# kshedden/muscato

Hardware: AMD Instinct MI355X
Metric: reads/sec (100 bp, multi-map) at 1/2/4/8 MI355X; confirm-kernel HBM GB/s vs peak (higher is better)
Workload: dtype u32

## Files before the change

include/muscato_hip.h:

```cpp
#ifndef MUSCATO_HIP_H
#define MUSCATO_HIP_H

#include <stdint.h>

#ifdef __cplusplus
extern "C" {
#endif

#define MUSC_ABI_VERSION 3
#define MUSC_MAX_WINDOWS 16

typedef struct musc_ctx musc_ctx;

typedef struct {
  uint32_t read_idx;
  uint32_t gene_idx;
  uint32_t pos;
  uint32_t nmiss;
} musc_hit;

typedef struct {
  int32_t n_windows;
  int32_t windows[MUSC_MAX_WINDOWS];
  int32_t window_width;
// ... 96 lines not shown
int musc_results_text(musc_ctx* ctx, uint64_t line0, uint64_t nlines, char* dst, uint64_t capacity, int dst_on_device,
                      uint64_t* nbytes);
int musc_results_last_ms(musc_ctx* ctx, float* ms_order, float* ms_text);
int musc_results_number_key(uint32_t pos, uint32_t nmiss, uint64_t* key);

enum { MUSC_SIDE_NONMATCH = 0, MUSC_SIDE_GENESTATS = 1, MUSC_SIDE_READSTATS = 2 };
int musc_side_prepare(musc_ctx* ctx, uint64_t* nrecords, uint64_t* nbytes);
int musc_side_text(musc_ctx* ctx, int which, uint64_t rec0, uint64_t nrec, char* dst, uint64_t capacity, int dst_on_device,
                   uint64_t* nbytes);
int musc_side_last_ms(musc_ctx* ctx, float* ms_prepare, float* ms_text);

#define MUSC_INSTANCE_WORDS 4
#define MUSC_INST_MATCH_T 1u
#define MUSC_INST_MATCH_G 2u
#define MUSC_INST_SCREEN 3u
#define MUSC_INST_SCREEN_T 4u
#define MUSC_INST_CONFIRM 5u
int musc_last_instance(const musc_ctx* ctx, uint32_t* out);
int musc_instances(uint32_t* out, uint32_t capacity, uint32_t* n);

int musc_stream_plan(uint64_t nreads, uint32_t fixed_len, uint32_t batch_reads, uint64_t* ends, uint8_t* is_batch_end,
                     uint64_t capacity, uint64_t* n, uint64_t* planned_batches);

int musc_overflow_probes(musc_ctx* ctx, uint32_t** read_idx, uint32_t** window, uint64_t* n);
void musc_free_u32(uint32_t* p);

#define MUSC_MM_MAX_READ_LEN 1024
int musc_maxmatches_apply(musc_ctx* ctx, int apply_mmtol, uint64_t* nhits, uint64_t* n_suspect_probes,
                          uint64_t* n_truncated_blocks);
int musc_maxmatches_last_ms(musc_ctx* ctx, float* ms);
int musc_maxmatches_last_detail(musc_ctx* ctx, uint64_t* n_pairs, float* ms_replay);

int musc_gather(musc_ctx* const* ctxs, int n, const uint64_t* read_base, musc_hit** hits,
                uint64_t* nhits);
int musc_gather_rccl(musc_ctx* const* ctxs, int n, const uint64_t* read_base, musc_hit** hits,
                     uint64_t* nhits);
int musc_rccl_probe(char* msg, uint64_t cap);

typedef struct musc_db_text_info {
  uint64_t n_targets, n_bases;
  uint64_t n_odd;
  uint32_t first_odd_target, reserved;
  uint64_t n_text_bytes, n_chunks;
  float ms_decode, ms_parse;
} musc_db_text_info;
int musc_sz_decode(musc_ctx* ctx, const uint8_t* bytes, uint64_t nbytes, uint8_t* dst, uint64_t capacity,
// ... 28 lines not shown
```

muscato_amd/_lib.py:

```python
from __future__ import annotations

import ctypes
import os

HERE = os.path.dirname(os.path.abspath(__file__))
LIB_PATH = os.environ.get("MUSC_LIB_PATH") or os.path.join(HERE, "libmuscato_hip.so")

MUSC_MAX_WINDOWS = 16


class MuscHit(ctypes.Structure):
    _fields_ = [("read_idx", ctypes.c_uint32), ("gene_idx", ctypes.c_uint32),
                ("pos", ctypes.c_uint32), ("nmiss", ctypes.c_uint32)]


class MuscParams(ctypes.Structure):
    _fields_ = [
        ("n_windows", ctypes.c_int32),
        ("windows", ctypes.c_int32 * MUSC_MAX_WINDOWS),
        ("window_width", ctypes.c_int32),
        ("pmatch", ctypes.c_double),
        ("min_dinuc", ctypes.c_int32),
        ("max_read_length", ctypes.c_int32),
        ("max_matches", ctypes.c_int32),
# ... 39 lines not shown
        ("n_targets", ctypes.c_uint64), ("n_bases", ctypes.c_uint64), ("n_odd", ctypes.c_uint64),
        ("first_odd_target", ctypes.c_uint32), ("reserved", ctypes.c_uint32),
        ("n_text_bytes", ctypes.c_uint64), ("n_chunks", ctypes.c_uint64),
        ("ms_decode", ctypes.c_float), ("ms_parse", ctypes.c_float),
    ]


class MuscTargetsPrepInfo(ctypes.Structure):
    _fields_ = [
        ("n_lines", ctypes.c_uint64), ("n_records", ctypes.c_uint64), ("n_targets", ctypes.c_uint64),
        ("n_dropped", ctypes.c_uint64), ("stop_line", ctypes.c_uint64), ("n_subx", ctypes.c_uint64),
        ("n_seq_bytes", ctypes.c_uint64), ("n_id_bytes", ctypes.c_uint64),
        ("ms", ctypes.c_float), ("reserved", ctypes.c_uint32),
    ]


SYMBOLS = [
    "musc_abi_version", "musc_init", "musc_destroy", "musc_last_error", "musc_reload_env",
    "musc_db_load_ascii", "musc_db_load_packed", "musc_db_build_index", "musc_db_build_index_for",
    "musc_db_set_partition_bases", "musc_db_partitions",
    "musc_reads_load_ascii", "musc_reads_load_packed", "musc_reads_load_packed32", "musc_reads_sort_unique",
    "musc_reads_prep_fastq", "musc_fastq_prep_free",
    "musc_match_device", "musc_hits_copy", "musc_hits_copy_packed", "musc_hits_copy_compact", "musc_hits_unpack", "musc_match", "musc_free_hits",
    "musc_get_stats", "musc_last_instance", "musc_instances", "musc_stream_plan", "musc_gather", "musc_gather_rccl", "musc_rccl_probe", "musc_overflow_probes", "musc_free_u32",
    "musc_results_set_gene_text", "musc_results_set_read_text", "musc_results_order", "musc_results_hits", "musc_results_text",
    "musc_results_last_ms", "musc_results_number_key",
    "musc_side_prepare", "musc_side_text", "musc_side_last_ms",
    "musc_maxmatches_apply", "musc_maxmatches_last_ms", "musc_maxmatches_last_detail",
    "musc_sz_decode", "musc_db_load_text",
    "musc_targets_prep", "musc_targets_prep_text", "musc_targets_prep_load", "musc_targets_prep_free", "musc_sz_frame",
]

SIDE_NONMATCH, SIDE_GENESTATS, SIDE_READSTATS = 0, 1, 2

_lib = None


def load() -> ctypes.CDLL:
    global _lib
    if _lib is not None:
        return _lib
    if not os.path.exists(LIB_PATH):
        raise ImportError(
            "muscato_amd: %s is missing -- build it with `python -m muscato_amd.build` "
            "(hipcc, gfx950).  There is no CPU fallback." % LIB_PATH)
    import sys
    torch = sys.modules.get("torch")
# ... 22 lines not shown
    lib.musc_db_set_partition_bases.argtypes = [vp, u64]
    lib.musc_db_partitions.argtypes = [vp, vp, ctypes.c_uint32, ctypes.POINTER(ctypes.c_uint32)]
    lib.musc_reads_load_ascii.argtypes = [vp, vp, vp, u64, ctypes.c_int]
    lib.musc_reads_load_packed.argtypes = [vp, vp, vp, vp, u64]
    lib.musc_reads_load_packed32.argtypes = [vp, vp, vp, vp, ctypes.c_uint32, u64, ctypes.c_int]
    lib.musc_reads_sort_unique.argtypes = [vp, vp, vp, u64, ctypes.c_int, ctypes.POINTER(vp), ctypes.POINTER(vp),
                                           ctypes.POINTER(u64)]
    lib.musc_reads_prep_fastq.argtypes = [vp, vp, u64, ctypes.c_int, i32, i32, ctypes.POINTER(MuscFastqPrep)]
    lib.musc_reads_prep_fastq.restype = ctypes.c_int
    lib.musc_fastq_prep_free.argtypes = [ctypes.POINTER(MuscFastqPrep)]
    lib.musc_fastq_prep_free.restype = None
    lib.musc_match_device.argtypes = [vp, ctypes.POINTER(MuscParams), ctypes.POINTER(u64)]
    lib.musc_hits_copy.argtypes = [vp, vp, u64, ctypes.c_int]
    lib.musc_hits_copy_packed.argtypes = [vp, vp, u64, ctypes.c_int, u64, ctypes.POINTER(i32)]
    lib.musc_hits_copy_compact.argtypes = [vp, vp, u64, vp, u64, ctypes.c_int, ctypes.POINTER(i32)]
    lib.musc_hits_unpack.argtypes = [vp, vp, u64, ctypes.c_int, ctypes.POINTER(i32), vp]
    lib.musc_match.argtypes = [vp, ctypes.POINTER(MuscParams), ctypes.POINTER(vp), ctypes.POINTER(u64)]
    lib.musc_free_hits.argtypes = [vp]
    lib.musc_free_hits.restype = None
    lib.musc_get_stats.argtypes = [vp, ctypes.POINTER(MuscStats)]
    lib.musc_last_instance.argtypes = [vp, ctypes.POINTER(ctypes.c_uint32)]
    lib.musc_instances.argtypes = [ctypes.POINTER(ctypes.c_uint32), ctypes.c_uint32, ctypes.POINTER(ctypes.c_uint32)]
    lib.musc_stream_plan.argtypes = [u64, ctypes.c_uint32, ctypes.c_uint32, vp, vp, u64, ctypes.POINTER(u64), ctypes.POINTER(u64)]
    lib.musc_overflow_probes.argtypes = [vp, ctypes.POINTER(vp), ctypes.POINTER(vp), ctypes.POINTER(u64)]
    lib.musc_overflow_probes.restype = ctypes.c_int
    lib.musc_free_u32.argtypes = [vp]
    lib.musc_free_u32.restype = None
    lib.musc_gather.argtypes = [ctypes.POINTER(vp), ctypes.c_int, ctypes.POINTER(u64),
                                ctypes.POINTER(vp), ctypes.POINTER(u64)]
    lib.musc_gather_rccl.argtypes = lib.musc_gather.argtypes
    lib.musc_rccl_probe.argtypes = [ctypes.c_char_p, ctypes.c_uint64]
    lib.musc_results_set_gene_text.argtypes = [vp, vp, vp, vp, ctypes.c_uint32]
    lib.musc_results_set_read_text.argtypes = [vp, vp, vp, u64]
    lib.musc_results_order.argtypes = [vp, vp, u64, ctypes.c_int, ctypes.POINTER(u64), ctypes.POINTER(u64)]
    lib.musc_results_hits.argtypes = [vp, vp, u64, ctypes.c_int]
    lib.musc_results_text.argtypes = [vp, u64, u64, vp, u64, ctypes.c_int, ctypes.POINTER(u64)]
    lib.musc_results_last_ms.argtypes = [vp, ctypes.POINTER(ctypes.c_float), ctypes.POINTER(ctypes.c_float)]
    lib.musc_results_number_key.argtypes = [ctypes.c_uint32, ctypes.c_uint32, ctypes.POINTER(u64)]
    lib.musc_side_prepare.argtypes = [vp, ctypes.POINTER(u64), ctypes.POINTER(u64)]
    lib.musc_side_text.argtypes = [vp, ctypes.c_int, u64, u64, vp, u64, ctypes.c_int, ctypes.POINTER(u64)]
    lib.musc_side_last_ms.argtypes = [vp, ctypes.POINTER(ctypes.c_float), ctypes.POINTER(ctypes.c_float)]
    lib.musc_maxmatches_apply.argtypes = [vp, ctypes.c_int, ctypes.POINTER(u64), ctypes.POINTER(u64), ctypes.POINTER(u64)]
    lib.musc_maxmatches_apply.restype = ctypes.c_int
    lib.musc_maxmatches_last_ms.argtypes = [vp, ctypes.POINTER(ctypes.c_float)]
    lib.musc_maxmatches_last_ms.restype = ctypes.c_int
    lib.musc_maxmatches_last_detail.argtypes = [vp, ctypes.POINTER(u64), ctypes.POINTER(ctypes.c_float)]
# ... 25 lines not shown
```

muscato_amd/api.py:

```python
from __future__ import annotations

import ctypes
import json
from dataclasses import dataclass, field, asdict
from typing import List, Optional, Sequence, Tuple

import numpy as np

from . import _lib


class MuscatoError(RuntimeError):
    pass


@dataclass
class DbTextInfo:
    n_targets: int
    n_bases: int
    n_odd: int
    first_odd_target: int
    n_text_bytes: int
    n_chunks: int
    ms_decode: float
# ... 542 lines not shown
def instances() -> List[dict]:
    lib = _lib.load()
    n = ctypes.c_uint32()
    if lib.musc_instances(None, 0, ctypes.byref(n)):
        raise RuntimeError("musc_instances failed")
    buf = (ctypes.c_uint32 * max(1, n.value))()
    lib.musc_instances(buf, n.value, ctypes.byref(n))
    return [decode_instance(w) for w in buf[:n.value]]


def stream_plan(nreads: int, fixed_len: int, batch_reads: int = 16 << 20) -> dict:
    lib = _lib.load()
    n, planned = ctypes.c_uint64(), ctypes.c_uint64()
    if lib.musc_stream_plan(nreads, fixed_len, batch_reads, None, None, 0, ctypes.byref(n), ctypes.byref(planned)):
        raise ValueError("musc_stream_plan: %d reads of %d bases is not a read set the loader takes" % (nreads, fixed_len))
    ends = np.zeros(max(1, n.value), dtype=np.uint64)
    flags = np.zeros(max(1, n.value), dtype=np.uint8)
    lib.musc_stream_plan(nreads, fixed_len, batch_reads, ends.ctypes.data, flags.ctypes.data, n.value, ctypes.byref(n),
                         ctypes.byref(planned))
    ends, flags = ends[:n.value], flags[:n.value]
    return {"piece_ends": ends, "batch_ends": ends[flags != 0], "planned_batches": int(planned.value)}


def gather(engines: Sequence["Engine"], read_bases: Sequence[int], rccl: bool = False) -> np.ndarray:
    lib = engines[0]._lib
    n = len(engines)
    arr = (ctypes.c_void_p * n)(*[e._h for e in engines])
    bases = (ctypes.c_uint64 * n)(*[int(b) for b in read_bases])
    ph, cnt = ctypes.c_void_p(), ctypes.c_uint64()
    rc = lib.musc_gather_rccl(arr, n, bases, ctypes.byref(ph), ctypes.byref(cnt)) if rccl else 1
    if rccl and rc == 2:
        raise MuscatoError("musc_gather_rccl failed (%d): %s" % (rc, lib.musc_last_error(engines[0]._h).decode()))
    if rc != 0:
        rc = lib.musc_gather(arr, n, bases, ctypes.byref(ph), ctypes.byref(cnt))
    if rc != 0:
        raise MuscatoError("musc_gather failed (%d): %s" % (rc, lib.musc_last_error(engines[0]._h).decode()))
    out = np.zeros((cnt.value, 4), dtype=np.uint32)
    if cnt.value:
        ctypes.memmove(out.ctypes.data, ph, cnt.value * 16)
    lib.musc_free_hits(ph)
    return out


def sorted_hits(a: np.ndarray) -> np.ndarray:
    if len(a) == 0:
        return a.reshape(0, 4)
# ... 3 lines not shown
```

muscato_amd/csrc/kernels_index.hpp:

```cpp
#pragma once

typedef uint32_t u32x4_v __attribute__((ext_vector_type(4)));
#define BUCKET_INLINE 3
struct __attribute__((aligned(64))) Bucket {
  static constexpr uint32_t NIN = BUCKET_INLINE;
  uint32_t count;
  uint32_t cursor;
  uint64_t ovf;
  uint4 e[BUCKET_INLINE];
  __device__ uint64_t ovf_entry(uint32_t slot) const { return ovf + (slot - NIN); }
  __device__ static uint64_t ovf_units(uint32_t count) { return count > NIN ? count - NIN : 0u; }
  __device__ void set_ovf(uint64_t v) { ovf = v; }
};
static_assert(sizeof(Bucket) == 64, "bucket must be half a cache line");

#define LINE_INLINE 7
struct __attribute__((aligned(128))) LineBucket {
  static constexpr uint32_t NIN = LINE_INLINE;
  uint32_t count;
  uint32_t ovf;
  uint32_t cursor;
  uint32_t pad;
  uint4 e[LINE_INLINE];
  __device__ uint64_t ovf_entry(uint32_t slot) const { return (uint64_t)ovf * 8u + (slot - NIN); }
// ... 41 lines not shown
      const uint32_t slot = atomicAdd(&T[b].cursor, 1u);
      const uint64_t rem = e - g;
      const uint32_t lr = (uint32_t)(jx > 65535 ? 65535 : jx) | ((uint32_t)(rem > 65535 ? 65535 : rem) << 16);
      const uint32_t fl = flank_left(db2, g) | (((uint32_t)ext64(db2, 2 * (g + (uint64_t)ww)) & 0xFFFFu) << 16);
      const uint4 ent = make_uint4(wide ? (gene | ((uint32_t)(g >> 32) << 24)) : gene, (uint32_t)g, lr, fl);
      if (slot < BT::NIN) T[b].e[slot] = ent;
      else E[T[b].ovf_entry(slot)] = ent;
    }
  }
}

template <class BT>
__global__ void k_index_ovf_count(const BT* __restrict__ T, uint64_t nb, uint64_t* __restrict__ tmp) {
  const uint64_t b = (uint64_t)blockIdx.x * blockDim.x + threadIdx.x;
  if (b < nb) tmp[b] = BT::ovf_units(T[b].count);
  else if (b == nb) tmp[b] = 0;
}

template <class BT>
__global__ void k_index_ovf_set(BT* __restrict__ T, uint64_t nb, const uint64_t* __restrict__ tmp) {
  const uint64_t b = (uint64_t)blockIdx.x * blockDim.x + threadIdx.x;
  if (b < nb) T[b].set_ovf(tmp[b]);
}
```

muscato_amd/csrc/kernels_match.hpp:

```cpp
#pragma once

#define CTX_BASES 120
#define CTX_INLINE 3
#define CTX_MAX_W 4
#define CTX_XFLAG 0x80000000u
#define CTX_XMANY 0xFFu
#define CTX_XNONE 0xFFu

struct __attribute__((aligned(128))) CtxBucket {
  uint32_t count;
  uint32_t ovf;
  uint32_t gene[CTX_INLINE];
  uint32_t jx[CTX_INLINE];
  uint32_t ctx[CTX_INLINE][8];
};
static_assert(sizeof(CtxBucket) == 128, "a context bucket is one cache line");

struct CtxEntry {
  uint32_t gene, jx;
  uint32_t ctx[8];
};
static_assert(sizeof(CtxEntry) == 40, "overflow entries are packed");

#define CTXW_BASES 200
// ... 49 lines not shown
  uint64_t bo = 2 * g;
  int left = 2 * (int)n;
  while (left > 0) {
    const int take = left < 64 ? left : 64;
    if (ext64(dbm2, bo) & lowmask64(take)) return true;
    bo += 64;
    left -= 64;
  }
  return false;
}

DEV uint32_t ctx_xtail(uint32_t w, uint32_t xtail) {
  const uint32_t rem = w >> 16;
  return (w & 0xFFFFu) | ((rem > 255u ? 255u : rem) << 16) | ((xtail & 0xFFu) << 24);
}
DEV uint32_t ctx_rem(uint32_t w, bool flagged) { return flagged ? (w >> 16) & 0xFFu : w >> 16; }

template <bool SCATTER, bool WIDE>
__global__ __launch_bounds__(256) void k_index_ctx(const uint32_t* __restrict__ db2, const uint32_t* __restrict__ dbm2,
                                                   const uint32_t* __restrict__ dbx,
                                                   const uint64_t* __restrict__ seq_off, uint32_t nseq,
                                                   uint64_t nbases, uint64_t g_lo, uint64_t g_hi, int ww, int bits,
                                                   int direct, int CL, CtxBucket* __restrict__ T, void* __restrict__ Ev,
                                                   uint32_t* __restrict__ cursor) {
  __shared__ uint32_t s_g0;
  const uint64_t nchunks = (g_hi - g_lo + blockDim.x - 1) / blockDim.x;
  for (uint64_t chunk = blockIdx.x; chunk < nchunks; chunk += gridDim.x) {
    const uint64_t gfirst = g_lo + chunk * blockDim.x;
    __syncthreads();
    if (threadIdx.x == 0) {
      uint32_t lo = 0, hi = nseq;
      while (hi - lo > 1) {
        const uint32_t mid = lo + (hi - lo) / 2;
        if (seq_off[mid] <= gfirst) lo = mid; else hi = mid;
      }
      s_g0 = lo;
    }
    __syncthreads();
    const uint64_t g = gfirst + threadIdx.x;
    if (g >= g_hi) continue;
    uint32_t gene = s_g0;
    while (seq_off[gene + 1] <= g) gene++;
    const uint64_t s = seq_off[gene], e = seq_off[gene + 1];
    const uint64_t jx = g - s;
    if (jx + (uint64_t)ww > e - s) continue;
    uint32_t xflag = 0, xgene = 0, xtail = 0;
    if (dbx) {
// ... 9 lines not shown
        for (int j = 0; j < (NB + 15) / 16; j++) {
          uint32_t m = (uint32_t)ext64s(dbm2, 2 * lo + 32 * j) & 0x55555555u & bit_range_mask(2 * tlo - 32 * j, 2 * thi - 32 * j);
          nx += (uint32_t)__popc(m);
          if (m && where2 == CTX_XNONE) {
            const uint32_t p = 16u * (uint32_t)j + (((uint32_t)__ffs(m) - 1u) >> 1);
            if (nx == (uint32_t)__popc(m)) {
              where = p;
              m &= m - 1u;
              if (m) where2 = 16u * (uint32_t)j + (((uint32_t)__ffs(m) - 1u) >> 1);
            } else {
              where2 = p;
            }
          }
        }
        if (nx) {
          xflag = CTX_XFLAG;
          xgene = (nx <= 2 ? where : CTX_XMANY) << 24;
          xtail = 0x100u | where2;
        }
      }
    }
    const uint32_t b = bucket_of(db2, nullptr, 2 * g, ww, bits, direct);
    if (!SCATTER) {
      atomicAdd(&T[b].count, 1u);
    } else {
      const uint32_t slot = atomicAdd(&cursor[b], 1u);
      if constexpr (WIDE) {
        CtxBucketW* const TW = reinterpret_cast<CtxBucketW*>(T);
        CtxEntryW ent;
        ent.gene = gene | xgene;
        ent.jx = (uint32_t)jx | xflag;
        ctx_words<CTXW_WORDS>(db2, g, e, CL, ent.ctx);
        if (xtail) ent.ctx[CTXW_WORDS - 1] = ctx_xtail(ent.ctx[CTXW_WORDS - 1], xtail);
        uint32_t* pw = slot < CTXW_INLINE ? reinterpret_cast<uint32_t*>(&TW[b].e[slot])
                                          : reinterpret_cast<uint32_t*>(Ev) + ctx_entry_word<true>(TW[b].ovf + (slot - CTXW_INLINE));
        pw[0] = ent.gene;
        pw[1] = ent.jx;
#pragma unroll
        for (int i = 0; i < CTXW_WORDS; i++) pw[2 + i] = ent.ctx[i];
      } else {
        uint32_t c[8];
        ctx_words<8>(db2, g, e, CL, c);
        if (xtail) c[7] = ctx_xtail(c[7], xtail);
        if (slot < CTX_INLINE) {
          T[b].gene[slot] = gene | xgene;
          T[b].jx[slot] = (uint32_t)jx | xflag;
          uint4* dst = reinterpret_cast<uint4*>(T[b].ctx[slot]);
          dst[0] = make_uint4(c[0], c[1], c[2], c[3]);
          dst[1] = make_uint4(c[4], c[5], c[6], c[7]);
        } else {
          uint32_t* p = reinterpret_cast<uint32_t*>(Ev) + ctx_entry_word<false>(T[b].ovf + (slot - CTX_INLINE));
          p[0] = gene | xgene;
          p[1] = (uint32_t)jx | xflag;
#pragma unroll
          for (int i = 0; i < 8; i++) p[2 + i] = c[i];
        }
      }
    }
  }
}

MUSC_KERNEL void k_ctx_ovf_count(const CtxBucket* __restrict__ T, uint64_t nb, uint32_t n_inline, uint64_t* __restrict__ tmp) {
  const uint64_t b = (uint64_t)blockIdx.x * blockDim.x + threadIdx.x;
  if (b < nb) {
    const uint32_t c = T[b].count;
    tmp[b] = c > n_inline ? c - n_inline : 0u;
  } else if (b == nb) {
    tmp[b] = 0;
  }
}

MUSC_KERNEL void k_ctx_ovf_set(CtxBucket* __restrict__ T, uint64_t nb, const uint64_t* __restrict__ tmp) {
  const uint64_t b = (uint64_t)blockIdx.x * blockDim.x + threadIdx.x;
  if (b < nb) T[b].ovf = (uint32_t)tmp[b];
}


struct MatchParams {
  int32_t W, ww, min_dinuc, bits, direct, mmtol, apply_mmtol, max_len, CL;
  uint32_t q1zero_mask;
  int32_t reserved0;
  int32_t win[CTX_MAX_W];
  const uint64_t* seq_off;
  const uint32_t* dbm2;
  uint32_t need[CTX_MAX_W];
  uint32_t wm[CTX_MAX_W][CTX_MAX_W][CTXW_WORDS];
  uint32_t lm[CTXW_BASES + 1][CTX_MAX_W][CTXW_WORDS];
};


inline void match_tables(MatchParams& mp) {
  for (int k = 0; k < CTX_MAX_W; k++) {
    mp.need[k] = 0;
    if (k >= mp.W) continue;
    const int sh = 2 * (mp.CL - mp.win[k]);
    mp.need[k] = ((1u << k) - 1u) | (mp.direct ? 0u : (1u << k));
    for (int kk = 0; kk < mp.W; kk++)
      for (int j = 0; j < CTXW_WORDS; j++)
// ... 160 lines not shown
```

muscato_amd/csrc/muscato_hip.hip:

```cpp

#include <hip/hip_runtime.h>
#include <rccl/rccl.h>
#include <dlfcn.h>

#include <algorithm>
#include <cstdarg>
#include <cstdio>
#include <cstdlib>
#include <cstring>
#include <map>
#include <mutex>
#include <string>
#include <type_traits>
#include <vector>

#include "../../include/muscato_hip.h"

#include "ctx_state.hpp"
#include "dev_mem.hpp"
#include "index_plan.hpp"
#include "load_plan.hpp"

#include "kernels_common.hpp"
#include "kernels_index.hpp"
#include "kernels_screen.hpp"
#include "kernels_confirm.hpp"
#include "kernels_match.hpp"
#include "kernels_match_lane_inst.hpp"
#include "kernels_screen_lane.hpp"
#include "kernels_partition.hpp"
#include "kernels_results.hpp"
#include "side_names.hpp"
#include "kernels_side.hpp"
#include "kernels_maxmatches.hpp"
#include "kernels_fastq.hpp"
MUSC_LANE_INSTANCES_4(extern)
MUSC_LANE_INSTANCES_8(extern)
MUSC_LANE_INSTANCES_12(extern)
MUSC_LANE_INSTANCES_8W(extern)
MUSC_LANE_INSTANCES_12W(extern)
MUSC_LANE_INSTANCES_16W(extern)
MUSC_LANE_INSTANCES_SPEC(extern)
MUSC_DMA_INSTANCES(extern)
// ... 1039 lines not shown
  *n = (uint32_t)ids.size();
  if (out)
    for (uint32_t i = 0; i < capacity && i < ids.size(); i++) out[i] = ids[i];
  return 0;
}

int musc_stream_plan(uint64_t nreads, uint32_t fixed_len, uint32_t batch_reads, uint64_t* ends, uint8_t* is_batch_end,
                     uint64_t capacity, uint64_t* n, uint64_t* planned_batches) {
  if (!n || fixed_len > 65535 || nreads >= 0xFFFFFFF0ull) return 1;
  if (batch_reads < 1 || batch_reads > (16u << 20)) batch_reads = 16u << 20;
  StreamPlan sp;
  stream_plan(nreads, batch_reads, &sp);
  *n = sp.piece_end.size();
  if (planned_batches) *planned_batches = std::max<uint64_t>(sp.batch_end.size(), 1);
  size_t b = 0;
  for (size_t i = 0; i < sp.piece_end.size() && i < capacity; i++) {
    if (ends) ends[i] = sp.piece_end[i];
    while (b < sp.batch_end.size() && sp.batch_end[b] < sp.piece_end[i]) b++;
    if (is_batch_end) is_batch_end[i] = b < sp.batch_end.size() && sp.batch_end[b] == sp.piece_end[i];
  }
  return 0;
}

int musc_gather(musc_ctx* const* ctxs, int n, const uint64_t* read_base, musc_hit** hits, uint64_t* nhits) {
  if (!ctxs || n < 1 || !hits || !nhits) return 1;
  uint64_t total = 0;
  for (int i = 0; i < n; i++) {
    if (!ctxs[i]) return 1;
    total += ctxs[i]->nhits;
  }
  musc_hit* h = (musc_hit*)malloc(sizeof(musc_hit) * (total ? total : 1));
  if (!h) return fail(ctxs[0], 7, "musc_gather: out of host memory");
  uint64_t o = 0;
  for (int i = 0; i < n; i++) {
    musc_ctx* c = ctxs[i];
    int rc = musc_hits_copy(c, h + o, c->nhits, 0);
    if (rc) {
      free(h);
      return rc;
    }
    const uint64_t base = read_base ? read_base[i] : 0;
    for (uint64_t j = 0; j < c->nhits; j++) h[o + j].read_idx += (uint32_t)base;
    o += c->nhits;
  }
  *hits = h;
  *nhits = total;
// ... 147 lines not shown
```

muscato_amd/csrc/muscato_index.hpp:

```cpp
#pragma once

namespace mi = musc_index;

static_assert(sizeof(Bucket) == mi::BUCKET_BYTES && sizeof(LineBucket) == mi::LINE_BUCKET_BYTES && sizeof(uint4) == mi::ENTRY_BYTES,
              "index_plan.hpp sizes the window-start index with these");
static_assert(sizeof(CtxBucket) == mi::CTX_BUCKET_BYTES && sizeof(CtxEntry) == mi::CTX_ENTRY_BYTES && sizeof(CtxEntryW) == mi::CTX_ENTRYW_BYTES,
              "index_plan.hpp sizes the context index with these");

namespace {

void free_index(musc_ctx* c) {
  c->idx = mi::Resident();
  c->st.index_freed();
}

struct IdxRange {
  uint32_t g0, g1;
  uint64_t b0, b1, size;
};
IdxRange whole_db(const musc_ctx* c) { return IdxRange{0, c->nseq, 0, c->nbases, c->nbases}; }

uint64_t index_avail(const musc_ctx* c) {
  size_t mfree = 0, mtotal = 0;
  if (hipMemGetInfo(&mfree, &mtotal) != hipSuccess) {
    (void)hipGetLastError();
    return 0;
  }
  return (uint64_t)mfree + c->idx_T.bytes + c->idx_E.bytes + c->ctx_T.bytes + c->ctx_E.bytes;
}

template <class Count, class Sizes, class Set, class Cap, class Fill>
int build_index_table(musc_ctx* c, int bits, uint64_t bucket_b, bool cursors, bool soft, DevMem& T, DevMem& E,
                      Count count, Sizes sizes, Set set, Cap cap, Fill fill) {
  const uint64_t nb = 1ull << bits;
  auto no_mem = [&](hipError_t e, const char* what) {
    (void)hipGetLastError();
    return soft ? 100 : fail(c, 10, "hipMalloc of %s failed: %s", what, hipGetErrorString(e));
  };
  c->ev_used = 0;
  hipEvent_t e0 = pool_event(c), e1 = pool_event(c), e2 = pool_event(c), e3 = pool_event(c);
  if (!e0 || !e1 || !e2 || !e3) return fail(c, 10, "hipEventCreate failed");
  hipError_t e = T.grow((nb + 1) * bucket_b);
  if (e != hipSuccess) return no_mem(e, "the index table");
  TmpBufs B, Bc;
  uint64_t *tmp = nullptr, *stmp = nullptr;
  uint32_t* cursor = nullptr;
  if ((e = B.alloc(&tmp, (nb + 1 + 16) * 8)) != hipSuccess || (e = B.alloc(&stmp, scan_tmp_elems(nb + 1) * 8)) != hipSuccess ||
      (cursors && (e = Bc.alloc(&cursor, (nb + 1) * 4)) != hipSuccess))
    return no_mem(e, "the index build's temporaries");
  HIPCHK(c, hipEventRecord(e0, c->stream));
  HIPCHK(c, hipMemsetAsync(T.p, 0, (nb + 1) * bucket_b, c->stream));
  if (cursor) HIPCHK(c, hipMemsetAsync(cursor, 0, (nb + 1) * 4, c->stream));
  count(cursor);
  HIPCHK(c, hipGetLastError());
  sizes(tmp);
  HIPCHK(c, hipGetLastError());
  int rc = scan_u64(c, tmp, tmp, nb + 1, stmp);
  if (rc) return rc;
  uint64_t novf = 0, e_bytes = 0;
  HIPCHK(c, hipMemcpyAsync(&novf, tmp + nb, 8, hipMemcpyDeviceToHost, c->stream));
  set(tmp);
  HIPCHK(c, hipGetLastError());
  HIPCHK(c, hipEventRecord(e2, c->stream));
  HIPCHK(c, hipStreamSynchronize(c->stream));
  B.release();
  if ((rc = cap(&novf, &e_bytes))) return rc;
  c->idx_novf = novf;
  if ((e = E.grow(e_bytes)) != hipSuccess) return no_mem(e, "the index's overflow entries");
  HIPCHK(c, hipEventRecord(e3, c->stream));
  fill(cursor);
  HIPCHK(c, hipGetLastError());
  HIPCHK(c, hipEventRecord(e1, c->stream));
  HIPCHK(c, hipStreamSynchronize(c->stream));
  float ms = 0, ms2 = 0;
  (void)hipEventElapsedTime(&ms, e0, e2);
  (void)hipEventElapsedTime(&ms2, e3, e1);
  c->stats.ms_index_build = ms + ms2;
  return 0;
}

template <class BT>
int build_window_index(musc_ctx* c, const mi::Resident& w, const IdxRange& R) {
  const uint64_t nb = 1ull << w.bits;
  const unsigned blocks = (unsigned)std::min<uint64_t>((R.b1 - R.b0 + 255) / 256, 1u << 22);
  auto T = [c] { return static_cast<BT*>(c->idx_T.p); };
  auto index = [&](auto filling, uint4* E) {
    if (R.b1 > R.b0)
      hipLaunchKernelGGL((k_index<decltype(filling)::value, BT>), dim3(blocks), dim3(256), 0, c->stream, c->db2, c->dbm2, c->seq_off, c->nseq,
                         R.b0, R.b1, w.ww, w.bits, w.direct, c->wide, T(), E);
  };
  return build_index_table(
      c, w.bits, sizeof(BT), false, false, c->idx_T, c->idx_E, [&](uint32_t*) { index(std::false_type{}, (uint4*)nullptr); },
      [&](uint64_t* tmp) { hipLaunchKernelGGL((k_index_ovf_count<BT>), dim3(nblk(nb + 1, 256)), dim3(256), 0, c->stream, T(), nb, tmp); },
      [&](uint64_t* tmp) { hipLaunchKernelGGL((k_index_ovf_set<BT>), dim3(nblk(nb, 256)), dim3(256), 0, c->stream, T(), nb, tmp); },
      [&](uint64_t* novf, uint64_t* bytes) {
        if (std::is_same<BT, LineBucket>::value) {
          if (*novf >= 0xFFFFFFF0ull) return fail(c, 5, "internal: %llu overflow lines do not fit 32-bit numbers", (unsigned long long)*novf);
          *novf *= 8;
        }
        *bytes = (*novf + 16) * sizeof(uint4);
        return 0;
      },
      [&](uint32_t*) { index(std::true_type{}, static_cast<uint4*>(c->idx_E.p)); });
}

int build_ctx_index(musc_ctx* c, const mi::Resident& w, const IdxRange& R) {
  const uint64_t nb = 1ull << w.bits;
  const bool wide = w.kind == mi::K_CTXW;
  const unsigned blocks = (unsigned)std::min<uint64_t>((R.b1 - R.b0 + 255) / 256, 1u << 22);
  const uint32_t* const xm2 = c->db_has_x ? c->dbm2 : nullptr;
  const uint32_t* const xbl = c->db_has_x ? c->dbx : nullptr;
  auto T = [c] { return static_cast<CtxBucket*>(c->ctx_T.p); };
  auto index = [&](auto kern, void* E, uint32_t* cursor) {
    if (R.b1 > R.b0)
      hipLaunchKernelGGL(kern, dim3(blocks), dim3(256), 0, c->stream, c->db2, xm2, xbl, c->seq_off, c->nseq, c->nbases, R.b0, R.b1, w.ww,
                         w.bits, w.direct, w.CL, T(), E, cursor);
  };
  return build_index_table(
      c, w.bits, sizeof(CtxBucket), true, true, c->ctx_T, c->ctx_E,
      [&](uint32_t* cursor) { index(k_index_ctx<false, false>, nullptr, cursor); },
      [&](uint64_t* tmp) {
        hipLaunchKernelGGL(k_ctx_ovf_count, dim3(nblk(nb + 1, 256)), dim3(256), 0, c->stream, T(), nb, (uint32_t)(wide ? CTXW_INLINE : CTX_INLINE), tmp);
      },
      [&](uint64_t* tmp) { hipLaunchKernelGGL(k_ctx_ovf_set, dim3(nblk(nb, 256)), dim3(256), 0, c->stream, T(), nb, tmp); },
      [&](uint64_t* novf, uint64_t* bytes) {
        if (*novf >= 0xFFFFFFF0ull) return fail(c, 5, "internal: %llu overflow entries do not fit 32-bit offsets", (unsigned long long)*novf);
        *bytes = ctx_entries_bytes(*novf + 16, wide);
        return 0;
      },
      [&](uint32_t* cursor) {
        if (wide) index(k_index_ctx<true, true>, c->ctx_E.p, cursor);
        else index(k_index_ctx<true, false>, c->ctx_E.p, cursor);
      });
}

int build_index(musc_ctx* c, const mi::Resident& want, const IdxRange& R) {
  free_index(c);
  int rc;
  if (mi::is_ctx(want.kind)) {
    c->idx_T.release();
    c->idx_E.release();
    rc = build_ctx_index(c, want, R);
  } else {
    c->ctx_T.release();
    c->ctx_E.release();
    rc = want.kind == mi::K_LINES ? build_window_index<LineBucket>(c, want, R) : build_window_index<Bucket>(c, want, R);
  }
  if (!rc) c->idx = want;
  return rc;
}

bool reads_xpos(musc_ctx* c, int wide) {
  if (c->rdx_of.gen == c->st.g.pass_inputs && c->rdx_of.wide == wide) return true;
  if (ensure(c, c->rdx, c->nreads)) return false;
  if (wide)
// ... 217 lines not shown
```

Before: 2.106 billion.

## Restructure context index build with separate counters, saved slots and vectorized table write

The context-index build now counts into a compact u32 counter array instead of atomically updating the bucket table. When the number of bases fits the bucket count, it records each entry's slot during the count pass so the fill pass can skip a second atomic. Overflow offsets are scanned in 32-bit and written into the table by one vectorized line-writer kernel, which replaces the old memset plus the two ovf-count and ovf-set kernels. This targets index-build memory traffic and atomic contention, at the cost of extra temporary memory for the slot array and a more complex build path.

```diff
diff --git a/include/muscato_hip.h b/include/muscato_hip.h
--- a/include/muscato_hip.h
+++ b/include/muscato_hip.h
@@ -142,6 +142,8 @@
 int musc_stream_plan(uint64_t nreads, uint32_t fixed_len, uint32_t batch_reads, uint64_t* ends, uint8_t* is_batch_end,
                      uint64_t capacity, uint64_t* n, uint64_t* planned_batches);
 
+int musc_index_build_plan(int32_t bits, uint64_t bases, uint64_t* out);
+
 int musc_overflow_probes(musc_ctx* ctx, uint32_t** read_idx, uint32_t** window, uint64_t* n);
 void musc_free_u32(uint32_t* p);
 
diff --git a/muscato_amd/_lib.py b/muscato_amd/_lib.py
--- a/muscato_amd/_lib.py
+++ b/muscato_amd/_lib.py
@@ -85,7 +85,7 @@
     "musc_reads_load_ascii", "musc_reads_load_packed", "musc_reads_load_packed32", "musc_reads_sort_unique",
     "musc_reads_prep_fastq", "musc_fastq_prep_free",
     "musc_match_device", "musc_hits_copy", "musc_hits_copy_packed", "musc_hits_copy_compact", "musc_hits_unpack", "musc_match", "musc_free_hits",
-    "musc_get_stats", "musc_last_instance", "musc_instances", "musc_stream_plan", "musc_gather", "musc_gather_rccl", "musc_rccl_probe", "musc_overflow_probes", "musc_free_u32",
+    "musc_get_stats", "musc_last_instance", "musc_instances", "musc_stream_plan", "musc_index_build_plan", "musc_gather", "musc_gather_rccl", "musc_rccl_probe", "musc_overflow_probes", "musc_free_u32",
     "musc_results_set_gene_text", "musc_results_set_read_text", "musc_results_order", "musc_results_hits", "musc_results_text",
     "musc_results_last_ms", "musc_results_number_key",
     "musc_side_prepare", "musc_side_text", "musc_side_last_ms",
@@ -154,6 +154,8 @@
     lib.musc_last_instance.argtypes = [vp, ctypes.POINTER(ctypes.c_uint32)]
     lib.musc_instances.argtypes = [ctypes.POINTER(ctypes.c_uint32), ctypes.c_uint32, ctypes.POINTER(ctypes.c_uint32)]
     lib.musc_stream_plan.argtypes = [u64, ctypes.c_uint32, ctypes.c_uint32, vp, vp, u64, ctypes.POINTER(u64), ctypes.POINTER(u64)]
+    lib.musc_index_build_plan.argtypes = [i32, u64, ctypes.POINTER(u64)]
+    lib.musc_index_build_plan.restype = ctypes.c_int
     lib.musc_overflow_probes.argtypes = [vp, ctypes.POINTER(vp), ctypes.POINTER(vp), ctypes.POINTER(u64)]
     lib.musc_overflow_probes.restype = ctypes.c_int
     lib.musc_free_u32.argtypes = [vp]
diff --git a/muscato_amd/api.py b/muscato_amd/api.py
--- a/muscato_amd/api.py
+++ b/muscato_amd/api.py
@@ -588,6 +588,16 @@
     return {"piece_ends": ends, "batch_ends": ends[flags != 0], "planned_batches": int(planned.value)}
 
 
+def index_build_plan(bits: int, bases: int) -> dict:
+    lib = _lib.load()
+    out = (ctypes.c_uint64 * 6)()
+    if lib.musc_index_build_plan(bits, bases, out):
+        raise ValueError("musc_index_build_plan: 2^%d buckets is no context table" % bits)
+    d = dict(zip(("slots", "cnt", "off", "slot", "before_entries", "at_fill"), (int(v) for v in out)))
+    d["slots"] = bool(d["slots"])
+    return d
+
+
 def gather(engines: Sequence["Engine"], read_bases: Sequence[int], rccl: bool = False) -> np.ndarray:
     lib = engines[0]._lib
     n = len(engines)
diff --git a/muscato_amd/csrc/host/index_build_plan_check.cpp b/muscato_amd/csrc/host/index_build_plan_check.cpp
--- /dev/null
+++ b/muscato_amd/csrc/host/index_build_plan_check.cpp
@@ -0,0 +1,57 @@
+#include <cstdio>
+#include <cstdlib>
+#include <random>
+
+#include "../index_build_plan.hpp"
+
+namespace {
+
+namespace mi = musc_index;
+
+int failures = 0;
+#define EXPECT(cond)                                              \
+  do {                                                            \
+    if (!(cond)) {                                                \
+      fprintf(stderr, "%s:%d: %s\n", __FILE__, __LINE__, #cond);  \
+      failures++;                                                 \
+    }                                                             \
+  } while (0)
+
+void check(int bits, uint64_t bases) {
+  const uint64_t nb = 1ull << bits;
+  const mi::BuildTemps t = mi::build_temps(bits, bases);
+  EXPECT(t.slots == (bases <= nb));
+  EXPECT(t.cnt == (nb + 1) * 4 && t.off == (nb + 1) * 4);
+  EXPECT(t.slot == (t.slots ? bases * 4 : 0u));
+  const uint64_t counted = mi::build_temps_counted(bits);
+  EXPECT(t.before_entries() <= counted);
+  EXPECT(t.at_fill() <= t.before_entries());
+  for (mi::Kind k : {mi::K_CTX, mi::K_CTXW})
+    EXPECT(counted <= mi::index_need(k, bits, bases) - (nb + 1) * mi::bucket_bytes(k));
+}
+
+}
+
+int main() {
+  check(30, 1000000000ull);
+  check(27, 100000000ull);
+  for (int bits = 8; bits <= 30; bits++) {
+    const uint64_t nb = 1ull << bits;
+    const uint64_t around[] = {0, 1, nb - 1, nb, nb + 1, 2 * nb, 9 * nb + 3};
+    for (uint64_t bases : around) check(bits, bases);
+  }
+  std::mt19937_64 rng(27);
+  for (int round = 0; round < 20000; round++) {
+    const int bits = 8 + (int)(rng() % 23);
+    check(bits, rng() % (12ull << bits));
+  }
+  EXPECT(!mi::build_temps(8, 200000).slots);
+  EXPECT(mi::build_temps(30, 1000000000ull).slots);
+  EXPECT(mi::build_temps(30, 1000000000ull).before_entries() == (1ull << 30) * 8 + 8 + 4000000000ull);
+  if (failures) {
+    fprintf(stderr, "%d checks failed\n", failures);
+    return 1;
+  }
+  puts("ok");
+  return 0;
+}
diff --git a/muscato_amd/csrc/index_build_plan.hpp b/muscato_amd/csrc/index_build_plan.hpp
--- /dev/null
+++ b/muscato_amd/csrc/index_build_plan.hpp
@@ -0,0 +1,28 @@
+#pragma once
+
+#include <cstdint>
+
+#include "index_plan.hpp"
+
+namespace musc_index {
+
+struct BuildTemps {
+  bool slots;
+  uint64_t cnt, off, slot;
+  uint64_t before_entries() const { return cnt + off + slot; }
+  uint64_t at_fill() const { return off + (slots ? slot : cnt); }
+};
+
+inline BuildTemps build_temps(int bits, uint64_t bases) {
+  const uint64_t nb1 = (1ull << bits) + 1;
+  BuildTemps t{};
+  t.slots = bases <= nb1 - 1;
+  t.cnt = nb1 * 4;
+  t.off = nb1 * 4;
+  t.slot = t.slots ? bases * 4 : 0;
+  return t;
+}
+
+inline uint64_t build_temps_counted(int bits) { return ((1ull << bits) + 1) * 12; }
+
+}
diff --git a/muscato_amd/csrc/kernels_index.hpp b/muscato_amd/csrc/kernels_index.hpp
--- a/muscato_amd/csrc/kernels_index.hpp
+++ b/muscato_amd/csrc/kernels_index.hpp
@@ -87,3 +87,30 @@
   const uint64_t b = (uint64_t)blockIdx.x * blockDim.x + threadIdx.x;
   if (b < nb) T[b].set_ovf(tmp[b]);
 }
+
+
+MUSC_KERNEL void k_index_zero(uint32_t* __restrict__ p, uint64_t n) {
+  const uint64_t stride = (uint64_t)gridDim.x * blockDim.x;
+  for (uint64_t i = (uint64_t)blockIdx.x * blockDim.x + threadIdx.x; i < n; i += stride) p[i] = 0u;
+}
+
+MUSC_KERNEL void k_ovf_sizes(const uint32_t* __restrict__ cnt, uint64_t nb, uint32_t n_inline, uint32_t* __restrict__ off) {
+  const uint64_t b = (uint64_t)blockIdx.x * blockDim.x + threadIdx.x;
+  if (b > nb) return;
+  const uint32_t c = b < nb ? cnt[b] : 0u;
+  off[b] = c > n_inline ? c - n_inline : 0u;
+}
+
+template <int PIECES, class Header>
+__global__ __launch_bounds__(256) void k_index_lines(u32x4_v* __restrict__ T, uint64_t nb, const uint32_t* __restrict__ cnt,
+                                                     const uint32_t* __restrict__ off) {
+  const uint64_t npieces = (nb + 1) * PIECES, stride = (uint64_t)gridDim.x * blockDim.x;
+  for (uint64_t i = (uint64_t)blockIdx.x * blockDim.x + threadIdx.x; i < npieces; i += stride) {
+    u32x4_v v = {0u, 0u, 0u, 0u};
+    if (i % PIECES == 0) {
+      const uint64_t b = i / PIECES;
+      if (b < nb) v = Header()(cnt[b], off[b]);
+    }
+    T[i] = v;
+  }
+}
diff --git a/muscato_amd/csrc/kernels_match.hpp b/muscato_amd/csrc/kernels_match.hpp
--- a/muscato_amd/csrc/kernels_match.hpp
+++ b/muscato_amd/csrc/kernels_match.hpp
@@ -95,7 +95,8 @@
                                                    const uint64_t* __restrict__ seq_off, uint32_t nseq,
                                                    uint64_t nbases, uint64_t g_lo, uint64_t g_hi, int ww, int bits,
                                                    int direct, int CL, CtxBucket* __restrict__ T, void* __restrict__ Ev,
-                                                   uint32_t* __restrict__ cursor) {
+                                                   uint32_t* __restrict__ cnt, uint32_t* __restrict__ slots,
+                                                   const uint32_t* __restrict__ off) {
   __shared__ uint32_t s_g0;
   const uint64_t nchunks = (g_hi - g_lo + blockDim.x - 1) / blockDim.x;
   for (uint64_t chunk = blockIdx.x; chunk < nchunks; chunk += gridDim.x) {
@@ -151,9 +152,10 @@
     }
     const uint32_t b = bucket_of(db2, nullptr, 2 * g, ww, bits, direct);
     if (!SCATTER) {
-      atomicAdd(&T[b].count, 1u);
+      const uint32_t slot = atomicAdd(&cnt[b], 1u);
+      if (slots) slots[g - g_lo] = slot;
     } else {
-      const uint32_t slot = atomicAdd(&cursor[b], 1u);
+      const uint32_t slot = slots ? slots[g - g_lo] : atomicAdd(&cnt[b], 1u);
       if constexpr (WIDE) {
         CtxBucketW* const TW = reinterpret_cast<CtxBucketW*>(T);
         CtxEntryW ent;
@@ -162,7 +164,7 @@
         ctx_words<CTXW_WORDS>(db2, g, e, CL, ent.ctx);
         if (xtail) ent.ctx[CTXW_WORDS - 1] = ctx_xtail(ent.ctx[CTXW_WORDS - 1], xtail);
         uint32_t* pw = slot < CTXW_INLINE ? reinterpret_cast<uint32_t*>(&TW[b].e[slot])
-                                          : reinterpret_cast<uint32_t*>(Ev) + ctx_entry_word<true>(TW[b].ovf + (slot - CTXW_INLINE));
+                                          : reinterpret_cast<uint32_t*>(Ev) + ctx_entry_word<true>(off[b] + (slot - CTXW_INLINE));
         pw[0] = ent.gene;
         pw[1] = ent.jx;
 #pragma unroll
@@ -178,7 +180,7 @@
           dst[0] = make_uint4(c[0], c[1], c[2], c[3]);
           dst[1] = make_uint4(c[4], c[5], c[6], c[7]);
         } else {
-          uint32_t* p = reinterpret_cast<uint32_t*>(Ev) + ctx_entry_word<false>(T[b].ovf + (slot - CTX_INLINE));
+          uint32_t* p = reinterpret_cast<uint32_t*>(Ev) + ctx_entry_word<false>(off[b] + (slot - CTX_INLINE));
           p[0] = gene | xgene;
           p[1] = (uint32_t)jx | xflag;
 #pragma unroll
@@ -189,20 +191,9 @@
   }
 }
 
-MUSC_KERNEL void k_ctx_ovf_count(const CtxBucket* __restrict__ T, uint64_t nb, uint32_t n_inline, uint64_t* __restrict__ tmp) {
-  const uint64_t b = (uint64_t)blockIdx.x * blockDim.x + threadIdx.x;
-  if (b < nb) {
-    const uint32_t c = T[b].count;
-    tmp[b] = c > n_inline ? c - n_inline : 0u;
-  } else if (b == nb) {
-    tmp[b] = 0;
-  }
-}
-
-MUSC_KERNEL void k_ctx_ovf_set(CtxBucket* __restrict__ T, uint64_t nb, const uint64_t* __restrict__ tmp) {
-  const uint64_t b = (uint64_t)blockIdx.x * blockDim.x + threadIdx.x;
-  if (b < nb) T[b].ovf = (uint32_t)tmp[b];
-}
+struct CtxHeader {
+  __device__ u32x4_v operator()(uint32_t count, uint32_t ovf) const { return u32x4_v{count, ovf, 0u, 0u}; }
+};
 
 
 struct MatchParams {
diff --git a/muscato_amd/csrc/muscato_hip.hip b/muscato_amd/csrc/muscato_hip.hip
--- a/muscato_amd/csrc/muscato_hip.hip
+++ b/muscato_amd/csrc/muscato_hip.hip
@@ -19,6 +19,7 @@
 #include "ctx_state.hpp"
 #include "dev_mem.hpp"
 #include "index_plan.hpp"
+#include "index_build_plan.hpp"
 #include "load_plan.hpp"
 
 #include "kernels_common.hpp"
@@ -1104,6 +1105,14 @@
   return 0;
 }
 
+int musc_index_build_plan(int32_t bits, uint64_t bases, uint64_t* out) {
+  if (!out || bits < 1 || bits > 30) return 1;
+  const musc_index::BuildTemps t = musc_index::build_temps(bits, bases);
+  const uint64_t v[6] = {t.slots ? 1u : 0u, t.cnt, t.off, t.slot, t.before_entries(), t.at_fill()};
+  std::copy(v, v + 6, out);
+  return 0;
+}
+
 int musc_gather(musc_ctx* const* ctxs, int n, const uint64_t* read_base, musc_hit** hits, uint64_t* nhits) {
   if (!ctxs || n < 1 || !hits || !nhits) return 1;
   uint64_t total = 0;
diff --git a/muscato_amd/csrc/muscato_index.hpp b/muscato_amd/csrc/muscato_index.hpp
--- a/muscato_amd/csrc/muscato_index.hpp
+++ b/muscato_amd/csrc/muscato_index.hpp
@@ -29,9 +29,64 @@
   return (uint64_t)mfree + c->idx_T.bytes + c->idx_E.bytes + c->ctx_T.bytes + c->ctx_E.bytes;
 }
 
+inline unsigned lines_grid(uint64_t npieces) { return (unsigned)std::min<uint64_t>((npieces + 255) / 256, 1u << 16); }
+
+template <class Count, class Sizes, class Lines, class Cap, class Fill>
+int build_index_table(musc_ctx* c, mi::Kind kind, int bits, uint64_t bases, bool soft, DevMem& T, DevMem& E, Count count, Sizes sizes,
+                      Lines lines, Cap cap, Fill fill) {
+  const uint64_t nb = 1ull << bits;
+  const mi::BuildTemps bt = mi::build_temps(bits, bases);
+  auto no_mem = [&](hipError_t e, const char* what) {
+    (void)hipGetLastError();
+    return soft ? 100 : fail(c, 10, "hipMalloc of %s failed: %s", what, hipGetErrorString(e));
+  };
+  c->ev_used = 0;
+  hipEvent_t e0 = pool_event(c), e1 = pool_event(c), e2 = pool_event(c), e3 = pool_event(c);
+  if (!e0 || !e1 || !e2 || !e3) return fail(c, 10, "hipEventCreate failed");
+  hipError_t e = T.grow((nb + 1) * mi::bucket_bytes(kind));
+  if (e != hipSuccess) return no_mem(e, "the index table");
+  TmpBufs B, K;
+  uint32_t *cnt = nullptr, *off = nullptr, *stmp = nullptr, *slot = nullptr;
+  if ((e = (bt.slots ? B : K).alloc(&cnt, bt.cnt)) != hipSuccess || (e = K.alloc(&off, bt.off + 64)) != hipSuccess ||
+      (e = B.alloc(&stmp, scan_tmp_elems(nb + 1) * 4)) != hipSuccess || (bt.slots && (e = K.alloc(&slot, bt.slot)) != hipSuccess))
+    return no_mem(e, "the index build's temporaries");
+  HIPCHK(c, hipEventRecord(e0, c->stream));
+  auto zero_cnt = [&] { hipLaunchKernelGGL(k_index_zero, dim3(lines_grid(nb + 1)), dim3(256), 0, c->stream, cnt, nb + 1); };
+  zero_cnt();
+  count(cnt, slot);
+  HIPCHK(c, hipGetLastError());
+  sizes(cnt, off);
+  HIPCHK(c, hipGetLastError());
+  int rc = scan_u32(c, off, off, nb + 1, false, stmp);
+  if (rc) return rc;
+  uint32_t total = 0;
+  HIPCHK(c, hipMemcpyAsync(&total, off + nb, 4, hipMemcpyDeviceToHost, c->stream));
+  lines(cnt, off);
+  HIPCHK(c, hipGetLastError());
+  HIPCHK(c, hipEventRecord(e2, c->stream));
+  HIPCHK(c, hipStreamSynchronize(c->stream));
+  B.release();
+  uint64_t novf = total, e_bytes = 0;
+  if ((rc = cap(&novf, &e_bytes))) return rc;
+  c->idx_novf = novf;
+  if ((e = E.grow(e_bytes)) != hipSuccess) return no_mem(e, "the index's overflow entries");
+  HIPCHK(c, hipEventRecord(e3, c->stream));
+  if (!bt.slots) zero_cnt();
+  fill(bt.slots ? nullptr : cnt, slot, off);
+  HIPCHK(c, hipGetLastError());
+  HIPCHK(c, hipEventRecord(e1, c->stream));
+  HIPCHK(c, hipStreamSynchronize(c->stream));
+  float ms = 0, ms2 = 0;
+  (void)hipEventElapsedTime(&ms, e0, e2);
+  (void)hipEventElapsedTime(&ms2, e3, e1);
+  c->stats.ms_index_build = ms + ms2;
+  return 0;
+}
+
 template <class Count, class Sizes, class Set, class Cap, class Fill>
-int build_index_table(musc_ctx* c, int bits, uint64_t bucket_b, bool cursors, bool soft, DevMem& T, DevMem& E,
-                      Count count, Sizes sizes, Set set, Cap cap, Fill fill) {
+int build_window_table(musc_ctx* c, int bits, uint64_t bucket_b, DevMem& T, DevMem& E, Count count, Sizes sizes, Set set, Cap cap,
+                       Fill fill) {
+  const bool soft = false;
   const uint64_t nb = 1ull << bits;
   auto no_mem = [&](hipError_t e, const char* what) {
     (void)hipGetLastError();
@@ -42,16 +97,13 @@
   if (!e0 || !e1 || !e2 || !e3) return fail(c, 10, "hipEventCreate failed");
   hipError_t e = T.grow((nb + 1) * bucket_b);
   if (e != hipSuccess) return no_mem(e, "the index table");
-  TmpBufs B, Bc;
+  TmpBufs B;
   uint64_t *tmp = nullptr, *stmp = nullptr;
-  uint32_t* cursor = nullptr;
-  if ((e = B.alloc(&tmp, (nb + 1 + 16) * 8)) != hipSuccess || (e = B.alloc(&stmp, scan_tmp_elems(nb + 1) * 8)) != hipSuccess ||
-      (cursors && (e = Bc.alloc(&cursor, (nb + 1) * 4)) != hipSuccess))
+  if ((e = B.alloc(&tmp, (nb + 1 + 16) * 8)) != hipSuccess || (e = B.alloc(&stmp, scan_tmp_elems(nb + 1) * 8)) != hipSuccess)
     return no_mem(e, "the index build's temporaries");
   HIPCHK(c, hipEventRecord(e0, c->stream));
   HIPCHK(c, hipMemsetAsync(T.p, 0, (nb + 1) * bucket_b, c->stream));
-  if (cursor) HIPCHK(c, hipMemsetAsync(cursor, 0, (nb + 1) * 4, c->stream));
-  count(cursor);
+  count();
   HIPCHK(c, hipGetLastError());
   sizes(tmp);
   HIPCHK(c, hipGetLastError());
@@ -68,7 +120,7 @@
   c->idx_novf = novf;
   if ((e = E.grow(e_bytes)) != hipSuccess) return no_mem(e, "the index's overflow entries");
   HIPCHK(c, hipEventRecord(e3, c->stream));
-  fill(cursor);
+  fill();
   HIPCHK(c, hipGetLastError());
   HIPCHK(c, hipEventRecord(e1, c->stream));
   HIPCHK(c, hipStreamSynchronize(c->stream));
@@ -89,8 +141,8 @@
       hipLaunchKernelGGL((k_index<decltype(filling)::value, BT>), dim3(blocks), dim3(256), 0, c->stream, c->db2, c->dbm2, c->seq_off, c->nseq,
                          R.b0, R.b1, w.ww, w.bits, w.direct, c->wide, T(), E);
   };
-  return build_index_table(
-      c, w.bits, sizeof(BT), false, false, c->idx_T, c->idx_E, [&](uint32_t*) { index(std::false_type{}, (uint4*)nullptr); },
+  return build_window_table(
+      c, w.bits, sizeof(BT), c->idx_T, c->idx_E, [&] { index(std::false_type{}, (uint4*)nullptr); },
       [&](uint64_t* tmp) { hipLaunchKernelGGL((k_index_ovf_count<BT>), dim3(nblk(nb + 1, 256)), dim3(256), 0, c->stream, T(), nb, tmp); },
       [&](uint64_t* tmp) { hipLaunchKernelGGL((k_index_ovf_set<BT>), dim3(nblk(nb, 256)), dim3(256), 0, c->stream, T(), nb, tmp); },
       [&](uint64_t* novf, uint64_t* bytes) {
@@ -101,7 +153,7 @@
         *bytes = (*novf + 16) * sizeof(uint4);
         return 0;
       },
-      [&](uint32_t*) { index(std::true_type{}, static_cast<uint4*>(c->idx_E.p)); });
+      [&] { index(std::true_type{}, static_cast<uint4*>(c->idx_E.p)); });
 }
 
 int build_ctx_index(musc_ctx* c, const mi::Resident& w, const IdxRange& R) {
@@ -111,26 +163,29 @@
   const uint32_t* const xm2 = c->db_has_x ? c->dbm2 : nullptr;
   const uint32_t* const xbl = c->db_has_x ? c->dbx : nullptr;
   auto T = [c] { return static_cast<CtxBucket*>(c->ctx_T.p); };
-  auto index = [&](auto kern, void* E, uint32_t* cursor) {
+  auto index = [&](auto kern, void* E, uint32_t* cnt, uint32_t* slot, const uint32_t* off) {
     if (R.b1 > R.b0)
       hipLaunchKernelGGL(kern, dim3(blocks), dim3(256), 0, c->stream, c->db2, xm2, xbl, c->seq_off, c->nseq, c->nbases, R.b0, R.b1, w.ww,
-                         w.bits, w.direct, w.CL, T(), E, cursor);
+                         w.bits, w.direct, w.CL, T(), E, cnt, slot, off);
   };
   return build_index_table(
-      c, w.bits, sizeof(CtxBucket), true, true, c->ctx_T, c->ctx_E,
-      [&](uint32_t* cursor) { index(k_index_ctx<false, false>, nullptr, cursor); },
-      [&](uint64_t* tmp) {
-        hipLaunchKernelGGL(k_ctx_ovf_count, dim3(nblk(nb + 1, 256)), dim3(256), 0, c->stream, T(), nb, (uint32_t)(wide ? CTXW_INLINE : CTX_INLINE), tmp);
+      c, w.kind, w.bits, R.b1 - R.b0, true, c->ctx_T, c->ctx_E,
+      [&](uint32_t* cnt, uint32_t* slot) { index(k_index_ctx<false, false>, nullptr, cnt, slot, nullptr); },
+      [&](const uint32_t* cnt, uint32_t* off) {
+        hipLaunchKernelGGL(k_ovf_sizes, dim3(nblk(nb + 1, 256)), dim3(256), 0, c->stream, cnt, nb, (uint32_t)(wide ? CTXW_INLINE : CTX_INLINE), off);
       },
-      [&](uint64_t* tmp) { hipLaunchKernelGGL(k_ctx_ovf_set, dim3(nblk(nb, 256)), dim3(256), 0, c->stream, T(), nb, tmp); },
+      [&](const uint32_t* cnt, const uint32_t* off) {
+        hipLaunchKernelGGL((k_index_lines<8, CtxHeader>), dim3(lines_grid((nb + 1) * 8)), dim3(256), 0, c->stream,
+                           static_cast<u32x4_v*>(c->ctx_T.p), nb, cnt, off);
+      },
       [&](uint64_t* novf, uint64_t* bytes) {
         if (*novf >= 0xFFFFFFF0ull) return fail(c, 5, "internal: %llu overflow entries do not fit 32-bit offsets", (unsigned long long)*novf);
         *bytes = ctx_entries_bytes(*novf + 16, wide);
         return 0;
       },
-      [&](uint32_t* cursor) {
-        if (wide) index(k_index_ctx<true, true>, c->ctx_E.p, cursor);
-        else index(k_index_ctx<true, false>, c->ctx_E.p, cursor);
+      [&](uint32_t* cnt, uint32_t* slot, const uint32_t* off) {
+        if (wide) index(k_index_ctx<true, true>, c->ctx_E.p, cnt, slot, off);
+        else index(k_index_ctx<true, false>, c->ctx_E.p, cnt, slot, off);
       });
 }
 
diff --git a/profiles/index_build.py b/profiles/index_build.py
--- /dev/null
+++ b/profiles/index_build.py
@@ -0,0 +1,79 @@
+#!/usr/bin/env python3
+import json
+import os
+import statistics
+import subprocess
+import sys
+import time
+
+ROOT = os.path.dirname(os.path.dirname(os.path.abspath(__file__)))
+OUT = os.path.join(ROOT, "profiles", "index_build.jsonl")
+
+
+def one(spec):
+    key, _, index = spec.partition(":")
+    if index:
+        os.environ["MUSC_INDEX"] = index
+    sys.path.insert(0, os.environ.get("MUSC_TREE", ROOT))
+    import torch
+    from muscato_amd import Config, Engine, synth
+    device = torch.device("cuda", 0)
+    wl = synth.workload_for(key, 1)
+    seed = synth.SEED_BASE + sum(ord(c) for c in wl.seed_key)
+    targets = synth.gen_targets(wl, device, seed)
+    toff = synth.offsets_for(wl.n_targets, wl.target_len, device)
+    torch.cuda.synchronize()
+    cfg = Config(Windows=list(wl.windows), WindowWidth=wl.window_width, PMatch=wl.pmatch, MinDinuc=wl.min_dinuc,
+                 MaxReadLength=wl.read_len, MaxMatches=wl.max_matches, MMTol=wl.mmtol, MatchMode=wl.match_mode)
+    with Engine(0) as eng:
+        eng.load_targets_device(targets.data_ptr(), toff.data_ptr(), wl.n_targets)
+        t0 = time.time()
+        eng.build_index_for(cfg, wl.read_len)
+        wall = time.time() - t0
+        st = eng.stats()
+    return {"workload": spec, "bases": wl.n_targets * wl.target_len, "ms_index_build": round(st["ms_index_build"], 3),
+            "index_build_wall_s": round(wall, 3)}
+
+
+def child(tree, spec):
+    env = dict(os.environ, MUSC_TREE=tree)
+    r = subprocess.run([sys.executable, os.path.abspath(__file__), "one", spec], env=env, stdout=subprocess.PIPE, stderr=subprocess.PIPE)
+    if r.returncode:
+        raise SystemExit("%s on %s failed (%d):\n%s" % (spec, tree, r.returncode, r.stderr.decode()[-2000:]))
+    return json.loads(r.stdout.decode().strip().splitlines()[-1])
+
+
+def ab(other, runs, specs):
+    sides = (("parent", os.path.abspath(other)), ("branch", ROOT))
+    with open(OUT, "a") as out:
+        def emit(rec):
+            out.write(json.dumps(rec) + "\n")
+            out.flush()
+            print(json.dumps(rec), flush=True)
+        for spec in specs:
+            ms = {name: [] for name, _ in sides}
+            wall = {name: [] for name, _ in sides}
+            for i in range(runs):
+                for name, tree in sides:
+                    rec = dict(child(tree, spec), side=name, run=i)
+                    ms[name].append(rec["ms_index_build"])
+                    wall[name].append(rec["index_build_wall_s"])
+                    emit(rec)
+            med = {k: statistics.median(v) for k, v in ms.items()}
+            spread = {k: round(max(v) - min(v), 3) for k, v in ms.items()}
+            diff = med["parent"] - med["branch"]
+            emit({"summary": True, "workload": spec, "runs": runs, "parent_ms": ms["parent"], "branch_ms": ms["branch"],
+                  "parent_median_ms": med["parent"], "branch_median_ms": med["branch"], "parent_spread_ms": spread["parent"],
+                  "branch_spread_ms": spread["branch"], "median_difference_ms": round(diff, 3),
+                  "parent_wall_median_s": statistics.median(wall["parent"]), "branch_wall_median_s": statistics.median(wall["branch"]),
+                  "faster_by_the_rule": diff > 5 * spread["parent"], "slower_by_the_rule": -diff > 5 * spread["branch"]})
+    return 0
+
+
+if __name__ == "__main__":
+    if len(sys.argv) >= 3 and sys.argv[1] == "one":
+        print(json.dumps(one(sys.argv[2])), flush=True)
+    elif len(sys.argv) >= 5 and sys.argv[1] == "ab":
+        sys.exit(ab(sys.argv[2], int(sys.argv[3]), sys.argv[4:]))
+    else:
+        sys.exit(__doc__)
```

Result: no change. 2.110 billion (median of 2 runs) (+0.2%).
